# speechcatcher-asr/statecatcher

Hardware: AMD Instinct MI355X
Metric: audio-frames/sec (LucyRNN+CTC, 80-d fbank, T=1500), whole job (higher is better)
Workload: dtype bf16

## Files before the change

### statecatcher_amd/csrc/lucy_scan.hip

```cpp

#include <atomic>
#include <initializer_list>
#include <type_traits>

#include "sc_common.h"

namespace sc {


constexpr int kChunk = 64;
typedef uint32_t v4u __attribute__((ext_vector_type(4)));
constexpr float kEps = 1e-6f;

struct ScanFwdArgs {
  const void* gates;
  const float* bias;
  const float* h0;
  const float* s0;
  void* out;
  float* s_out;
  float* h_out;
  float* ckpt;
  int B, T, D, nsc;
  int64_t g_bt, g_td, g_cd, g_cb, o_bt, o_bd;
  void* out_dup;
  void* out_lo;
  const float* ln_r;
  const float2* rec_in;
  float2* ln_stat;
  float2* rec_out;
  float ln_eps;
};

struct ScanBwdArgs {
  const void* gates;
  const float* bias;
  const float* ckpt;
  const void* dout;
  const float* ds_last;
  void* dgates;
  float* dh0;
  float* ds0;
  float* dbias;
  int B, T, D, nsc;
  int64_t g_bt, g_td, g_cd, g_cb, d_bt, d_bd, dg_bt, dg_td, dg_cd, dg_cb;
  const float* ln_r;
  const float2* ln_stat;
};

template <typename T, int PW> struct Pieces {
  static constexpr int EPP = PW / (int)sizeof(T);
  static constexpr int PPR = 64 / EPP;
  static_assert(EPP >= 1 && 64 % EPP == 0, "piece width");
};
template <typename T, int PW> struct LdsElem {
  static constexpr int BYTES = PW == 2 ? 4 : (int)sizeof(T);
  static __device__ __forceinline__ T get(const unsigned char* slot, int idx) {
    return *(const T*)(slot + idx * BYTES);
  }
};

__device__ __forceinline__ void step_terms(float r, float z, float k, float v, float hp, float dc,
                                           float al, float& zg, float& dec, float& u, float& hn) {
  const float rc2 = (r * r + z * z) * 0.5f + kEps;
  const float q = (k * k + v * v) * 0.5f + kEps;
  zg = sigm(z * rsq(rc2));
  dec = sigm(dc * rsq(dc * dc + kEps));
  const float alp = sigm(al * rsq(al * al + kEps));
  hn = hp * rsq(hp * hp + kEps);
  const float iq = rsq(q);
  const float kv = (k * iq) * (v * iq) * rcp(q + kEps);
  u = alp * kv;
}

typedef float f2 __attribute__((ext_vector_type(2)));
__device__ __forceinline__ f2 rsq2(f2 x) { return f2{rsq(x.x), rsq(x.y)}; }
__device__ __forceinline__ f2 rcp2(f2 x) { return f2{rcp(x.x), rcp(x.y)}; }
__device__ __forceinline__ f2 sigm2(f2 x) {
  const f2 t = x * f2{-kLog2e, -kLog2e};
  return rcp2(f2{1.0f, 1.0f} + f2{exp2_(t.x), exp2_(t.y)});
}
__device__ __forceinline__ f2 tanh2(f2 x) {
  const f2 t = x * f2{-2.0f * kLog2e, -2.0f * kLog2e};
  const f2 r = rcp2(f2{1.0f, 1.0f} + f2{exp2_(t.x), exp2_(t.y)});
  return r + r - f2{1.0f, 1.0f};
}
template <int DT> struct Pair {
  using T = typename Elem<DT>::T;
  typedef T t2 __attribute__((ext_vector_type(2)));
  static __device__ __forceinline__ t2 st(f2 v) { return __builtin_convertvector(v, t2); }
};

__device__ __forceinline__ void step_terms2(f2 r, f2 z, f2 k, f2 v, f2 hp, f2 dc, f2 al, f2& zg,
                                            f2& dec, f2& u, f2& hn) {
  const f2 eps = {kEps, kEps}, half = {0.5f, 0.5f};
  const f2 rc2 = (r * r + z * z) * half + eps;
  const f2 q = (k * k + v * v) * half + eps;
  zg = sigm2(z * rsq2(rc2));
  dec = sigm2(dc * rsq2(dc * dc + eps));
  const f2 alp = sigm2(al * rsq2(al * al + eps));
  hn = hp * rsq2(hp * hp + eps);
  const f2 iq = rsq2(q);
  u = alp * ((k * iq) * (v * iq) * rcp2(q + eps));
}

__device__ __forceinline__ float tanh_sig(float x) { return sigm(2.0f * x) * 2.0f - 1.0f; }

__device__ __forceinline__ void gate_grads(float r, float z, float k, float v, float hp, float dc,
                                           float al, float zg, float dec, float gh, float dpre,
                                           float gs, float hprev, float sprev, float c,
                                           float (&o)[7]) {
  const float rc2 = (r * r + z * z) * 0.5f + kEps;
  const float irc = rsq(rc2);
  const float ird = rsq(dc * dc + kEps);
  const float ira = rsq(al * al + kEps);
  const float alp = sigm(al * ira);
  const float irh = rsq(hp * hp + kEps);
  const float q = (k * k + v * v) * 0.5f + kEps;
  const float iq = rsq(q);
  const float iqe = rcp(q + kEps);
  const float d_zn = gh * (hprev - c) * zg * (1.0f - zg) * (irc * irc * irc);
  o[0] = -d_zn * z * r * 0.5f;
  o[1] = d_zn * (r * r * 0.5f + kEps);
  const float d_kv = gs * alp;
  const float f = iq * iq * iqe;
  const float fp = -(2.0f * q + kEps) * f * f;
  o[2] = d_kv * v * (f + k * k * fp);
  o[3] = d_kv * k * (f + v * v * fp);
  o[4] = dpre * kEps * (irh * irh * irh);
  o[5] = gs * sprev * dec * (1.0f - dec) * kEps * (ird * ird * ird);
  o[6] = gs * (k * v * f) * alp * (1.0f - alp) * kEps * (ira * ira * ira);
}


__device__ __forceinline__ void gate_grads2(f2 r, f2 z, f2 k, f2 v, f2 hp, f2 dc, f2 al, f2 zg,
                                            f2 dec, f2 gh, f2 dpre, f2 gs, f2 hprev, f2 sprev,
                                            f2 c, f2 (&o)[7]) {
  const f2 one = {1.0f, 1.0f}, eps = {kEps, kEps}, half = {0.5f, 0.5f};
  const f2 rc2 = (r * r + z * z) * half + eps;
  const f2 irc = rsq2(rc2);
  const f2 ird = rsq2(dc * dc + eps);
  const f2 ira = rsq2(al * al + eps);
  const f2 alp = sigm2(al * ira);
  const f2 irh = rsq2(hp * hp + eps);
  const f2 q = (k * k + v * v) * half + eps;
  const f2 iq = rsq2(q);
  const f2 iqe = rcp2(q + eps);
  const f2 d_zn = gh * (hprev - c) * zg * (one - zg) * (irc * irc * irc);
  o[0] = -d_zn * z * r * half;
  o[1] = d_zn * (r * r * half + eps);
  const f2 d_kv = gs * alp;
  const f2 f = iq * iq * iqe;
  const f2 fp = -(q + q + eps) * f * f;
  o[2] = d_kv * v * (f + k * k * fp);
  o[3] = d_kv * k * (f + v * v * fp);
  o[4] = dpre * eps * (irh * irh * irh);
  o[5] = gs * sprev * dec * (one - dec) * eps * (ird * ird * ird);
  o[6] = gs * (k * v * f) * alp * (one - alp) * eps * (ira * ira * ira);
}

__device__ __forceinline__ void step_terms_bwd2(f2 r, f2 z, f2 k, f2 v, f2 hp, f2 dc, f2 al,
                                                f2& zg, f2& dec, f2& u, f2& hn, f2 (&cf)[7]) {
  const f2 one = {1.0f, 1.0f}, eps = {kEps, kEps}, half = {0.5f, 0.5f};
  const f2 rc2 = (r * r + z * z) * half + eps;
  const f2 q = (k * k + v * v) * half + eps;
  const f2 irc = rsq2(rc2);
  zg = sigm2(z * irc);
  const f2 ird = rsq2(dc * dc + eps);
  dec = sigm2(dc * ird);
  const f2 ira = rsq2(al * al + eps);
  const f2 alp = sigm2(al * ira);
  const f2 irh = rsq2(hp * hp + eps);
  hn = hp * irh;
  const f2 iq = rsq2(q);
  const f2 f = iq * iq * rcp2(q + eps);
  const f2 kv = k * v * f;
  u = alp * kv;
  const f2 kz = zg * (one - zg) * (irc * irc * irc);
  cf[0] = -kz * z * r * half;
  cf[1] = kz * (r * r * half + eps);
  const f2 fp = -(q + q + eps) * f * f;
  cf[2] = alp * v * (f + k * k * fp);
  cf[3] = alp * k * (f + v * v * fp);
  cf[4] = eps * (irh * irh * irh);
  cf[5] = dec * (one - dec) * eps * (ird * ird * ird);
  cf[6] = kv * alp * (one - alp) * eps * (ira * ira * ira);
}

template <int NW>
__device__ __forceinline__ float compose_prefix(const float2 (*agg)[64], int lane, int w, float x) {
  int q = 0;
  for (; q + 4 <= w; q += 4) {
    const float2 m0 = agg[q][lane], m1 = agg[q + 1][lane], m2 = agg[q + 2][lane],
                 m3 = agg[q + 3][lane];
    x = fmaf(m0.x, x, m0.y);
    x = fmaf(m1.x, x, m1.y);
    x = fmaf(m2.x, x, m2.y);
    x = fmaf(m3.x, x, m3.y);
  }
  for (; q < w; ++q) {
    const float2 m = agg[q][lane];
    x = fmaf(m.x, x, m.y);
  }
  return x;
}
template <int NW>
__device__ __forceinline__ float compose_suffix(const float2 (*agg)[64], int lane, int w, float x) {
  int q = NW - 1;
  for (; q - 4 >= w; q -= 4) {
    const float2 m0 = agg[q][lane], m1 = agg[q - 1][lane], m2 = agg[q - 2][lane],
                 m3 = agg[q - 3][lane];
    x = fmaf(m0.x, x, m0.y);
    x = fmaf(m1.x, x, m1.y);
    x = fmaf(m2.x, x, m2.y);
    x = fmaf(m3.x, x, m3.y);
  }
  for (; q > w; --q) {
    const float2 m = agg[q][lane];
    x = fmaf(m.x, x, m.y);
  }
  return x;
}

template <int N>
__device__ __forceinline__ float group_sum_dpp(float x) {
  static_assert(N == 2 || N == 4 || N == 8 || N == 16, "group of 2..16 lanes");
  x = dpp_step<0xB1, 0xf, false>(x);
  if constexpr (N >= 4) x = dpp_step<0x4E, 0xf, false>(x);
  if constexpr (N >= 8) x = dpp_step<0x141, 0xf, false>(x);
  if constexpr (N >= 16) x = dpp_step<0x140, 0xf, false>(x);
  return x;
}

template <int DT, int NW, int LC, int PW, int FD, bool SPLIT = false, int LN = 0, int NB = 8>
__global__ void __launch_bounds__(NW * 64)
lucy_scan_fwd_kernel(ScanFwdArgs a) {
  static_assert(NW * LC == kChunk, "super-chunk must be 64 steps");
  using E = Elem<DT>;
  using T = typename E::T;
  using P = Pieces<T, PW>;
  constexpr int ROWS = LC * 7;
  constexpr int PIECES = ROWS * P::PPR;
  constexpr int NI = (PIECES + 63) / 64;
  const int lane = threadIdx.x & 63;
  const int w = uniform(threadIdx.x >> 6);
  const int b = blockIdx.y;
  const int blk = blockIdx.x;
  const int d = blk * 64 + lane;
  const bool dok = d < a.D;
  const int dc = dok ? d : a.D - 1;
  const int pcmax = (min(64, a.D - blk * 64) - 1) / P::EPP;

  extern __shared__ __attribute__((aligned(16))) unsigned char dyn_lds[];
  __shared__ float2 aggS[NW][64];
  __shared__ float2 aggH[NW][64];
  __shared__ float carS[2][64];
  __shared__ float carH[2][64];
  constexpr int RECN = (LN & 1) ? LC * NB : 2;
  static_assert(!(LN & 1) || (RECN <= 64 && NB % 2 == 0), "LN fold: LC * NB <= 64, NB even");
  __shared__ __attribute__((aligned(16))) float2 recS[(LN & 1) ? FD : 1][(LN & 1) ? NW : 1][RECN];
  using L = LdsElem<T, PW>;
  constexpr int SLOTB = ROWS * 64 * L::BYTES;
  const unsigned char* slots = dyn_lds + w * FD * SLOTB;
  const uint32_t slots_lds = lds_addr(slots);

  const T* gsrc = (const T*)a.gates + (int64_t)b * a.g_bt + (int64_t)blk * a.g_cb;
  const Buf<T> obuf((T*)a.out + (int64_t)b * a.o_bt);
  const Buf<T> dbuf(SPLIT ? (T*)a.out_dup + (int64_t)b * a.o_bt : (T*)a.out);
  const Buf<T> lbuf(SPLIT ? (T*)a.out_lo + (int64_t)b * a.o_bt : (T*)a.out);
  const uint32_t vo = (uint32_t)d * sizeof(T);
  const uint32_t otd = (uint32_t)(a.o_bd * sizeof(T));
  if (w == 0) {
    carS[0][lane] = dok ? a.s0[(int64_t)b * a.D + d] : 0.0f;
    carH[0][lane] = dok ? a.h0[(int64_t)b * a.D + d] : 0.0f;
  }
  float gb[7], fr[7];
#pragma unroll
  for (int g = 0; g < 7; ++g) {
    gb[g] = a.bias ? a.bias[g * a.D + dc] : 0.0f;
    fr[g] = (LN & 1) ? a.ln_r[g * a.D + dc] : 0.0f;
  }
  settle(gb);
  settle(fr);
  const int Tm1 = a.T - 1;
  auto issue_rec = [&](int k) __attribute__((always_inline)) {
    if constexpr ((LN & 1) != 0) {
      constexpr int NP = LC * NB / 2;
      if (lane < NP) {
        const int j = lane / (NB / 2), q2 = lane % (NB / 2);
        const int t = min(k * kChunk + w * LC + j, Tm1);
        dma_to_lds<16>(a.rec_in + ((int64_t)b * a.T + t) * NB + 2 * q2,
                       lds_addr(&recS[(LN & 1) ? k % FD : 0][(LN & 1) ? w : 0][0]));
      }
    }
  };
  auto issue = [&](int k) __attribute__((always_inline)) {
    issue_rec(k);
#pragma unroll
    for (int i = 0; i < NI; ++i) {
      const int p = i * 64 + lane;
      if (PIECES % 64 == 0 || p < PIECES) {
        const int row = p / P::PPR, pc = p % P::PPR;
        const int j = row / 7, g = row - 7 * (row / 7);
        const int t = min(k * kChunk + w * LC + j, Tm1);
        dma_to_lds<PW>(gsrc + (int64_t)t * a.g_td + (int64_t)g * a.g_cd + min(pc, pcmax) * P::EPP,
                       slots_lds + (uint32_t)((k % FD) * SLOTB) + i * 64 * (PW == 2 ? 4 : PW));
      }
    }
  };
  constexpr bool kFast = NI <= 16;
  uint32_t voff[kFast ? NI : 1];
#pragma unroll
  for (int i = 0; i < (kFast ? NI : 0); ++i) {
    const int p = min(i * 64 + lane, PIECES - 1);
    const int row = p / P::PPR, pc = p % P::PPR;
    voff[i] = (uint32_t)((row / 7) * a.g_td + (row % 7) * a.g_cd + min(pc, pcmax) * P::EPP) *
              (uint32_t)sizeof(T);
  }
  auto issue_next = [&](int k) __attribute__((always_inline)) {
    if (kFast && (k + 1) * kChunk <= a.T) {
      issue_rec(k);
      const T* gt = gsrc + ((int64_t)k * kChunk + w * LC) * a.g_td;
#pragma unroll
      for (int i = 0; i < (kFast ? NI : 0); ++i)
        if (PIECES % 64 == 0 || i * 64 + lane < PIECES)
          dma_to_lds_s<PW>(gt, voff[i], slots_lds + (uint32_t)((k % FD) * SLOTB) + i * 64 * (PW == 2 ? 4 : PW));
    } else {
      issue(k);
    }
  };
  constexpr int NIR = NI + ((LN & 1) ? 1 : 0);
  auto wait_next = [&](int k) __attribute__((always_inline)) {
    if (FD == 2 && k + 2 < a.nsc) dma_wait_younger<NIR>();
    else dma_wait();
  };
  if (a.nsc > 0) issue(0);
  if (FD == 2 && a.nsc > 1) issue(1);
  wait_next(-1);
  lds_barrier();
  auto chunk = [&](int k, auto fullc) __attribute__((always_inline)) {
    constexpr bool FULL = decltype(fullc)::value;
    constexpr int LP = LC / 2;
    const int t0 = k * kChunk + w * LC;
    f2 zg[LP], dec[LP], u[LP], x[LP], wz[LP];
    float gv[LC][7];
    const unsigned char* slot = slots + (k % FD) * SLOTB;
    if constexpr ((LN & 1) != 0) {
      const float2 rq = recS[(LN & 1) ? k % FD : 0][(LN & 1) ? w : 0][lane % RECN];
      const float mean = group_sum_dpp<NB>(rq.x) * (1.0f / NB);
      const float dm = rq.x - mean;
      const float m2 = group_sum_dpp<NB>(fmaf(64.0f * dm, dm, rq.y));
      const float rstd = rsq(m2 * (1.0f / (64 * NB)) + a.ln_eps);
      if (a.ln_stat && blk == 0 && lane % NB == 0 && lane < RECN && k * kChunk + w * LC + lane / NB < a.T)
        a.ln_stat[(int64_t)b * a.T + k * kChunk + w * LC + lane / NB] = make_float2(rstd, mean);
#pragma unroll
      for (int j = 0; j < LC; ++j) {
        const float rs = __int_as_float(__builtin_amdgcn_readlane(__float_as_int(rstd), j * NB));
        const float mu = __int_as_float(__builtin_amdgcn_readlane(__float_as_int(mean), j * NB));
        const float rm = -rs * mu;
#pragma unroll
        for (int g = 0; g < 7; ++g)
          gv[j][g] = fmaf(E::ld(L::get(slot, (j * 7 + g) * 64 + lane)), rs, fmaf(rm, fr[g], gb[g]));
      }
    } else {
#pragma unroll
      for (int j = 0; j < LC; ++j)
#pragma unroll
        for (int g = 0; g < 7; ++g) gv[j][g] = E::ld(L::get(slot, (j * 7 + g) * 64 + lane)) + gb[g];
    }
    lds_read_wait();
    if (k + FD < a.nsc) issue_next(k + FD);
#pragma unroll
    for (int p = 0; p < LP; ++p) {
      const int j = 2 * p;
      step_terms2(f2{gv[j][0], gv[j + 1][0]}, f2{gv[j][1], gv[j + 1][1]},
                  f2{gv[j][2], gv[j + 1][2]}, f2{gv[j][3], gv[j + 1][3]},
                  f2{gv[j][4], gv[j + 1][4]}, f2{gv[j][5], gv[j + 1][5]},
                  f2{gv[j][6], gv[j + 1][6]}, zg[p], dec[p], u[p], x[p]);
      if constexpr (!FULL) {
#pragma unroll
        for (int h2 = 0; h2 < 2; ++h2) {
          if (t0 + j + h2 >= a.T) {
            zg[p][h2] = 1.0f; dec[p][h2] = 1.0f; u[p][h2] = 0.0f; x[p][h2] = 0.0f;
          }
        }
      }
    }
    float As = 1.0f, Bs = 0.0f;
#pragma unroll
    for (int j = 0; j < LC; ++j) {
      As *= dec[j >> 1][j & 1];
      Bs = fmaf(dec[j >> 1][j & 1], Bs, u[j >> 1][j & 1]);
    }
    aggS[w][lane] = make_float2(As, Bs);
    lds_barrier();
    float s = carS[k & 1][lane];
    const float s_in = s;
    s = compose_prefix<NW>(aggS, lane, w, s);
#pragma unroll
    for (int j = 0; j < LC; ++j) {
      s = fmaf(dec[j >> 1][j & 1], s, u[j >> 1][j & 1]);
      x[j >> 1][j & 1] += s;
    }
#pragma unroll
    for (int p = 0; p < LP; ++p) {
      x[p] = tanh2(x[p]);
      wz[p] = x[p] - zg[p] * x[p];
    }
    float Ah = 1.0f, Bh = 0.0f;
#pragma unroll
    for (int j = 0; j < LC; ++j) {
      Ah *= zg[j >> 1][j & 1];
      Bh = fmaf(zg[j >> 1][j & 1], Bh, wz[j >> 1][j & 1]);
    }
    if (w == NW - 1) carS[(k + 1) & 1][lane] = s;
    aggH[w][lane] = make_float2(Ah, Bh);
    lds_barrier();
    float h = carH[k & 1][lane];
    const float h_in = h;
    h = compose_prefix<NW>(aggH, lane, w, h);
    float hs[LC];
#pragma unroll
    for (int j = 0; j < LC; ++j) {
      h = fmaf(zg[j >> 1][j & 1], h, wz[j >> 1][j & 1]);
      hs[j] = h;
    }
    if (w == NW - 1) carH[(k + 1) & 1][lane] = h;
    wait_next(k);
    if (w == 0 && a.ckpt && dok) {
      a.ckpt[((int64_t)(b * a.nsc + k) * 2) * a.D + d] = s_in;
      a.ckpt[((int64_t)(b * a.nsc + k) * 2 + 1) * a.D + d] = h_in;
    }
#pragma unroll
    for (int j = 0; j < LC; ++j)
      if (FULL || (dok && t0 + j < a.T)) {
        const T hi = E::st(hs[j]);
        obuf.st(hi, vo, (uint32_t)(t0 + j) * otd);
        if constexpr (SPLIT) {
          dbuf.st(hi, vo, (uint32_t)(t0 + j) * otd);
          lbuf.st(E::st(hs[j] - E::ld(hi)), vo, (uint32_t)(t0 + j) * otd);
        }
      }
    if constexpr ((LN & 2) != 0) {
      static_assert(LC == 4, "record butterfly written for 4 steps per wave");
      float v[8], ref[LC];
#pragma unroll
      for (int j = 0; j < LC; ++j) {
        const float hb = E::ld(E::st(hs[j]));
        ref[j] = __int_as_float(__builtin_amdgcn_readfirstlane(__float_as_int(hb)));
        const float dl = hb - ref[j];
        v[2 * j] = dl;
        v[2 * j + 1] = dl * dl;
      }
      const bool b5 = lane & 32, b4 = lane & 16, b3 = lane & 8;
      float u4[4], u2[2];
#pragma unroll
      for (int i = 0; i < 4; ++i)
        u4[i] = (b5 ? v[i + 4] : v[i]) + __shfl_xor(b5 ? v[i] : v[i + 4], 32);
#pragma unroll
      for (int i = 0; i < 2; ++i)
        u2[i] = (b4 ? u4[i + 2] : u4[i]) + __shfl_xor(b4 ? u4[i] : u4[i + 2], 16);
      float y = (b3 ? u2[1] : u2[0]) + __shfl_xor(b3 ? u2[0] : u2[1], 8);
      y = group_sum_dpp<8>(y);
      const float ysq = __shfl_xor(y, 8);
      const int j = lane >> 4;
      const float r = j == 0 ? ref[0] : j == 1 ? ref[1] : j == 2 ? ref[2] : ref[3];
      if ((lane & 15) == 0 && t0 + j < a.T)
        a.rec_out[((int64_t)b * a.T + t0 + j) * NB + blk] =
            make_float2(fmaf(y, 1.0f / 64, r), fmaxf(ysq - y * y * (1.0f / 64), 0.0f));
    }
  };
  const bool blk_full = (blk + 1) * 64 <= a.D;
  for (int k = 0; k < a.nsc; ++k) {
    if (blk_full && (k + 1) * kChunk <= a.T)
      chunk(k, std::true_type{});
    else
      chunk(k, std::false_type{});
  }
  lds_barrier();
  if (w == 0 && dok) {
    a.s_out[(int64_t)b * a.D + d] = carS[a.nsc & 1][lane];
    if (a.h_out) a.h_out[(int64_t)b * a.D + d] = carH[a.nsc & 1][lane];
  }
}

template <int DT, int NW, int LC, int PW, int NBUF, bool WST, int LN = 0>
__global__ void __launch_bounds__(NW * 64)
lucy_scan_bwd_kernel(ScanBwdArgs a) {
  static_assert(NW * LC == kChunk, "super-chunk must be 64 steps");
  using E = Elem<DT>;
  using T = typename E::T;
  using P = Pieces<T, PW>;
  constexpr int GROWS = LC * 7;
  constexpr int ROWS = LC * 8;
  constexpr int PIECES = ROWS * P::PPR;
  constexpr int NI = (PIECES + 63) / 64;
  static_assert(!WST || (NBUF == 2 && PW == 16), "staged stores need two 16-bit slots");
  const int lane = threadIdx.x & 63;
  const int w = uniform(threadIdx.x >> 6);
  const int b = blockIdx.y;
  const int blk = blockIdx.x;
  const int d = blk * 64 + lane;
  const bool dok = d < a.D;
  const int dc = dok ? d : a.D - 1;
  const int pcmax = (min(64, a.D - blk * 64) - 1) / P::EPP;

  extern __shared__ __attribute__((aligned(16))) unsigned char dyn_lds[];
  __shared__ float2 aggA[NW][64];
  __shared__ float2 aggB[NW][64];
  __shared__ float2 aggC[NW][64];
  __shared__ float2 aggD[NW][64];
  __shared__ float carGh[2][64];
  __shared__ float carGs[2][64];
  __shared__ float ckS[2][2][64];
  static_assert(!LN || (NBUF == 2 && WST), "LN fold: 16-bit gates with staged stores");
  __shared__ __attribute__((aligned(16))) float2 stS[LN ? NBUF : 1][LN ? NW : 1][LN ? LC : 1];
  using L = LdsElem<T, PW>;
  unsigned char* slots = dyn_lds + w * NBUF * ROWS * 64 * L::BYTES;
  const uint32_t slots_lds = lds_addr(slots);

  const T* gsrc = (const T*)a.gates + (int64_t)b * a.g_bt + (int64_t)blk * a.g_cb;
  const T* dsrc = (const T*)a.dout + (int64_t)b * a.d_bt + (int64_t)blk * 64;
  const float* cksrc = a.ckpt + (int64_t)b * a.nsc * 2 * a.D + dc;
  const Buf<T> dgbuf((T*)a.dgates + (int64_t)b * a.dg_bt + (int64_t)blk * a.dg_cb);
  const uint32_t vo = (uint32_t)lane * sizeof(T);
  if (w == 0) {
    carGh[0][lane] = 0.0f;
    carGs[0][lane] = (a.ds_last && dok) ? a.ds_last[(int64_t)b * a.D + d] : 0.0f;
  }
  float gb[LN ? 1 : 7];
  __shared__ float2 fbS[LN ? 7 : 1][64];
  if constexpr (LN) {
    if (w < 7)
      fbS[LN ? w : 0][lane] = make_float2(a.bias[w * a.D + dc], LN == 1 ? a.ln_r[w * a.D + dc] : 0.0f);
  } else {
#pragma unroll
    for (int g = 0; g < 7; ++g) gb[g] = a.bias ? a.bias[g * a.D + dc] : 0.0f;
    settle(gb);
  }
  const int Tm1 = a.T - 1;
  auto issue_stat = [&](int it) __attribute__((always_inline)) {
    if constexpr (LN) {
      if (lane < 2 * LC) {
        const int k = a.nsc - 1 - it;
        const int t = min(k * kChunk + w * LC + (lane >> 1), Tm1);
        dma_to_lds<4>((const float*)(a.ln_stat + (int64_t)b * a.T + t) + (lane & 1),
                      lds_addr(&stS[LN ? it % NBUF : 0][LN ? w : 0][0]));
      }
    }
  };
  auto issue = [&](int it) __attribute__((always_inline)) {
    const int k = a.nsc - 1 - it;
    issue_stat(it);
    const uint32_t base = slots_lds + (uint32_t)((it % NBUF) * ROWS * 64 * L::BYTES);
#pragma unroll
    for (int i = 0; i < NI; ++i) {
      const int p = i * 64 + lane;
      if (PIECES % 64 == 0 || p < PIECES) {
        const int row = p / P::PPR, pc = p % P::PPR;
        const int col = min(pc, pcmax) * P::EPP;
        const T* src;
        if (row < GROWS) {
          const int j = row / 7, g = row - 7 * (row / 7);
          const int t = min(k * kChunk + w * LC + j, Tm1);
          src = gsrc + (int64_t)t * a.g_td + (int64_t)g * a.g_cd + col;
        } else {
          const int t = min(k * kChunk + w * LC + (row - GROWS), Tm1);
          src = dsrc + (int64_t)t * a.d_bd + col;
        }
        dma_to_lds<PW>(src, base + i * 64 * (PW == 2 ? 4 : PW));
      }
    }
    if (w == 0) {
      dma_to_lds<4>(cksrc + (int64_t)(k * 2) * a.D, lds_addr(&ckS[it & 1][0][0]));
      dma_to_lds<4>(cksrc + (int64_t)(k * 2 + 1) * a.D, lds_addr(&ckS[it & 1][1][0]));
    }
  };
  static_assert((GROWS * P::PPR) % 64 == 0 && PIECES % 64 == 0, "uniform row kind per DMA");
  constexpr int NIF = NI <= 16 ? NI : 1;
  const bool same_layout = NI <= 16 && a.dg_td == a.g_td && a.dg_cd == a.g_cd;
  __shared__ uint32_t voffT[NIF][64];
  if constexpr (NI <= 16) {
#pragma unroll
    for (int i = 0; i < NI; ++i) {
      if (i % NW != w) continue;
      const int p = i * 64 + lane;
      const int row = p / P::PPR, pc = p % P::PPR;
      const int col = min(pc, pcmax) * P::EPP;
      voffT[i][lane] = (uint32_t)(row < GROWS ? (row / 7) * a.g_td + (row % 7) * a.g_cd + col
                                              : (row - GROWS) * a.d_bd + col) *
                       (uint32_t)sizeof(T);
    }
  }
  auto issue_full = [&](int it) __attribute__((always_inline)) {
    const int k = a.nsc - 1 - it;
    issue_stat(it);
    const uint32_t base = slots_lds + (uint32_t)((it % NBUF) * ROWS * 64 * L::BYTES);
    const int64_t t = (int64_t)k * kChunk + w * LC;
    const T* gt = gsrc + t * a.g_td;
    const T* dt = dsrc + t * a.d_bd;
#pragma unroll
    for (int i = 0; i < NI; ++i)
      dma_to_lds_s<PW>((i * 64) / P::PPR < GROWS ? (const void*)gt : (const void*)dt, voffT[i][lane],
                       base + i * 64 * (PW == 2 ? 4 : PW));
    if (w == 0) {
      const float* ck = a.ckpt + ((int64_t)b * a.nsc + k) * 2 * a.D;
      dma_to_lds_s<4>(ck, (uint32_t)dc * 4u, lds_addr(&ckS[it & 1][0][0]));
      dma_to_lds_s<4>(ck + a.D, (uint32_t)dc * 4u, lds_addr(&ckS[it & 1][1][0]));
    }
  };
  auto issue_next = [&](int it) __attribute__((always_inline)) {
    if constexpr (NI <= 16) issue_full(it); else issue(it);
  };
  f2 bacc[7];
  float bacc1[7];
#pragma unroll
  for (int g = 0; g < 7; ++g) {
    bacc[g] = f2{0.0f, 0.0f};
    bacc1[g] = 0.0f;
  }
  if (a.nsc > 0) issue(0);
  dma_wait();
  lds_barrier();
  auto chunk = [&](int it, auto fullc) __attribute__((always_inline)) {
    constexpr bool FULL = decltype(fullc)::value;
    constexpr int LP = LC / 2;
    const int k = a.nsc - 1 - it;
    const int t0 = k * kChunk + w * LC;
    unsigned char* slot = slots + (it % NBUF) * ROWS * 64 * L::BYTES;
    if (NBUF == 2 && it + 1 < a.nsc) issue_next(it + 1);
    const float s_ck = ckS[it & 1][0][lane];
    const float h_ck = ckS[it & 1][1][lane];
    f2 zg[LP], dec[LP], u[LP], x[LP], dj[LP], sv[LP], hv[LP], wz[LP];
    f2 cf[LP][7];
    float rg[NBUF == 1 ? LC : 1][7];
#pragma unroll
    for (int p = 0; p < LP; ++p) {
      const int j = 2 * p;
      f2 g7[7];
      f2 lrs = {1.0f, 1.0f}, lrm = {0.0f, 0.0f};
      if constexpr (LN) {
        const float2 s0 = stS[LN ? it % NBUF : 0][LN ? w : 0][j];
        const float2 s1 = stS[LN ? it % NBUF : 0][LN ? w : 0][j + 1];
        lrs = f2{s0.x, s1.x};
        lrm = -lrs * f2{s0.y, s1.y};
      }
#pragma unroll
      for (int g = 0; g < 7; ++g) {
        const f2 raw = f2{E::ld(L::get(slot, (j * 7 + g) * 64 + lane)),
                          E::ld(L::get(slot, ((j + 1) * 7 + g) * 64 + lane))};
        if constexpr (LN == 1) {
          const float2 fb = fbS[LN ? g : 0][lane];
          g7[g] = raw * lrs + (lrm * f2{fb.y, fb.y} + f2{fb.x, fb.x});
        } else if constexpr (LN == 2) {
          const float fbx = fbS[LN ? g : 0][lane].x;
          g7[g] = raw + f2{fbx, fbx};
        } else {
          g7[g] = raw + gb[LN ? 0 : g];
        }
        if constexpr (NBUF == 1) {
          rg[j][g] = g7[g].x;
          rg[j + 1][g] = g7[g].y;
        }
      }
      if constexpr (NBUF == 2)
        step_terms_bwd2(g7[0], g7[1], g7[2], g7[3], g7[4], g7[5], g7[6], zg[p], dec[p], u[p],
                        x[p], cf[p]);
      else
        step_terms2(g7[0], g7[1], g7[2], g7[3], g7[4], g7[5], g7[6], zg[p], dec[p], u[p], x[p]);
      dj[p] = f2{E::ld(L::get(slot, (GROWS + j) * 64 + lane)),
                 E::ld(L::get(slot, (GROWS + j + 1) * 64 + lane))};
      if constexpr (!FULL) {
#pragma unroll
        for (int h2 = 0; h2 < 2; ++h2) {
          if (t0 + j + h2 >= a.T) {
            zg[p][h2] = 1.0f; dec[p][h2] = 1.0f; u[p][h2] = 0.0f; x[p][h2] = 0.0f;
            dj[p][h2] = 0.0f;
          }
        }
      }
    }
    f2* stash = (f2*)slot;
    if constexpr (NBUF == 2) {
#pragma unroll
      for (int p = 0; p < LP; ++p)
#pragma unroll
        for (int c = 0; c < 4; ++c) stash[(p * 4 + c) * 64 + lane] = cf[p][c];
    }
    float As = 1.0f, Bs = 0.0f;
#pragma unroll
    for (int j = 0; j < LC; ++j) {
      As *= dec[j >> 1][j & 1];
      Bs = fmaf(dec[j >> 1][j & 1], Bs, u[j >> 1][j & 1]);
    }
    if constexpr (NBUF == 1) {
      lds_read_wait();
      if (it + 1 < a.nsc) issue_next(it + 1);
    }
    float Ph = 1.0f, Qh = 0.0f;
#pragma unroll
    for (int j = LC - 1; j >= 0; --j) {
      Qh = zg[j >> 1][j & 1] * (dj[j >> 1][j & 1] + Qh);
      Ph *= zg[j >> 1][j & 1];
    }
    aggA[w][lane] = make_float2(As, Bs);
    aggC[w][lane] = make_float2(Ph, Qh);
    lds_barrier();
    float s = compose_prefix<NW>(aggA, lane, w, s_ck);
#pragma unroll
    for (int j = 0; j < LC; ++j) {
      sv[j >> 1][j & 1] = s;
      s = fmaf(dec[j >> 1][j & 1], s, u[j >> 1][j & 1]);
      x[j >> 1][j & 1] += s;
    }
#pragma unroll
    for (int p = 0; p < LP; ++p) {
      x[p] = tanh2(x[p]);
      wz[p] = x[p] - zg[p] * x[p];
      if constexpr (NBUF == 2) cf[p][5] *= sv[p];
    }
    float Ah = 1.0f, Bh = 0.0f;
#pragma unroll
    for (int j = 0; j < LC; ++j) {
      Ah *= zg[j >> 1][j & 1];
      Bh = fmaf(zg[j >> 1][j & 1], Bh, wz[j >> 1][j & 1]);
    }
    float C = compose_suffix<NW>(aggC, lane, w, carGh[it & 1][lane]);
#pragma unroll
    for (int j = LC - 1; j >= 0; --j) {
      u[j >> 1][j & 1] = dj[j >> 1][j & 1] + C;
      C = zg[j >> 1][j & 1] * u[j >> 1][j & 1];
    }
    if (w == 0) carGh[(it + 1) & 1][lane] = C;
    f2 dp[LP];
#pragma unroll
    for (int p = 0; p < LP; ++p) dp[p] = (u[p] - u[p] * zg[p]) * (f2{1.0f, 1.0f} - x[p] * x[p]);
    float Ps = 1.0f, Qs = 0.0f;
#pragma unroll
    for (int j = LC - 1; j >= 0; --j) {
      Qs = dec[j >> 1][j & 1] * (dp[j >> 1][j & 1] + Qs);
      Ps *= dec[j >> 1][j & 1];
    }
    aggB[w][lane] = make_float2(Ah, Bh);
    aggD[w][lane] = make_float2(Ps, Qs);
    dma_wait();
    lds_barrier();
    float h = compose_prefix<NW>(aggB, lane, w, h_ck);
#pragma unroll
    for (int j = 0; j < LC; ++j) {
      if constexpr (NBUF == 2)
        hv[j >> 1][j & 1] = u[j >> 1][j & 1] * (h - x[j >> 1][j & 1]);
      else
        hv[j >> 1][j & 1] = h;
      h = fmaf(zg[j >> 1][j & 1], h, wz[j >> 1][j & 1]);
    }
    float Cs = compose_suffix<NW>(aggD, lane, w, carGs[it & 1][lane]);
    f2 gsj[LP];
#pragma unroll
    for (int j = LC - 1; j >= 0; --j) {
      gsj[j >> 1][j & 1] = dp[j >> 1][j & 1] + Cs;
      Cs = dec[j >> 1][j & 1] * gsj[j >> 1][j & 1];
    }
#pragma unroll
    for (int p = 0; p < LP; ++p) {
      const int jp = 2 * p;
      f2 o[7];
      if constexpr (NBUF == 2) {
        const f2 gz = hv[p];
        o[0] = gz * stash[(p * 4 + 0) * 64 + lane];
        o[1] = gz * stash[(p * 4 + 1) * 64 + lane];
        o[2] = gsj[p] * stash[(p * 4 + 2) * 64 + lane];
        o[3] = gsj[p] * stash[(p * 4 + 3) * 64 + lane];
        o[4] = dp[p] * cf[p][4];
        o[5] = gsj[p] * cf[p][5];
        o[6] = gsj[p] * cf[p][6];
      } else {
        f2 g7[7];
#pragma unroll
        for (int g = 0; g < 7; ++g) g7[g] = f2{rg[jp][g], rg[jp + 1][g]};
        gate_grads2(g7[0], g7[1], g7[2], g7[3], g7[4], g7[5], g7[6], zg[p], dec[p], u[p], dp[p],
                    gsj[p], hv[p], sv[p], x[p], o);
      }
      if constexpr (FULL && NBUF == 2) {
#pragma unroll
        for (int g = 0; g < 7; ++g) bacc[g] += o[g];
      }
      f2 lrs = {1.0f, 1.0f};
      if constexpr (LN) {
        lrs = f2{stS[LN ? it % NBUF : 0][LN ? w : 0][jp].x, stS[LN ? it % NBUF : 0][LN ? w : 0][jp + 1].x};
        if constexpr (FULL) {
#pragma unroll
          for (int g = 0; g < 7; ++g) o[g] *= lrs;
        }
      }
      if constexpr (FULL && WST) {
#pragma unroll
        for (int g = 0; g < 7; ++g) {
          const auto pr = Pair<DT>::st(o[g]);
          ((T*)slot)[(jp * 7 + g) * 64 + lane] = pr.x;
          ((T*)slot)[((jp + 1) * 7 + g) * 64 + lane] = pr.y;
        }
      } else {
#pragma unroll
        for (int h2 = 0; h2 < 2; ++h2) {
          const int j = jp + h2;
          if (FULL || (dok && t0 + j < a.T)) {
            const uint32_t so = (uint32_t)((t0 + j) * a.dg_td * sizeof(T));
#pragma unroll
            for (int g = 0; g < 7; ++g) {
              const float og = o[g][h2];
              const T ogt = E::st(LN ? og * lrs[h2] : og);
              if constexpr (WST) ((T*)slot)[(j * 7 + g) * 64 + lane] = ogt;
              else dgbuf.st(ogt, vo, so + (uint32_t)(g * a.dg_cd * sizeof(T)));
              if constexpr (NBUF == 1) bacc1[g] += E::ld(ogt);
              else if constexpr (!FULL) bacc[g][h2] += og;
            }
          }
        }
      }
    }
    if constexpr (WST) {
      constexpr int SP = LC * 7 * 8;
#pragma unroll
      for (int i = 0; i < (SP + 63) / 64; ++i) {
        const int p = i * 64 + lane;
        if (SP % 64 == 0 || p < SP) {
          const int row = p >> 3, pc = p & 7;
          const int j = row / 7, g = row - 7 * (row / 7);
          if (FULL || (t0 + j < a.T && pc <= pcmax)) {
            const v4u v = *(const v4u*)(slot + p * 16);
            if constexpr (FULL)
              __builtin_amdgcn_raw_buffer_store_b128(v, dgbuf.r, voffT[i][lane],
                                                     (uint32_t)(t0 * a.dg_td * sizeof(T)), 0);
            else
              __builtin_amdgcn_raw_buffer_store_b128(
                  v, dgbuf.r,
                  ((uint32_t)(t0 + j) * (uint32_t)a.dg_td + (uint32_t)g * (uint32_t)a.dg_cd +
                   (uint32_t)pc * 8u) * (uint32_t)sizeof(T),
                  0, 0);
          }
        }
      }
    }
    if (w == 0) carGs[(it + 1) & 1][lane] = Cs;
  };
  const bool blk_full = (blk + 1) * 64 <= a.D && (!WST || same_layout);
  for (int it = 0; it < a.nsc; ++it) {
    if constexpr (NBUF == 2) {
      if (blk_full && (a.nsc - it) * kChunk <= a.T) {
        chunk(it, std::true_type{});
        continue;
      }
    }
    chunk(it, std::false_type{});
  }
  lds_barrier();
  if (w == 0 && dok) {
    a.dh0[(int64_t)b * a.D + d] = carGh[a.nsc & 1][lane];
    a.ds0[(int64_t)b * a.D + d] = carGs[a.nsc & 1][lane];
  }
  if (a.dbias) {
#pragma unroll
    for (int g = 0; g < 7; ++g) {
      aggA[w][lane].x = NBUF == 1 ? bacc1[g] : bacc[g].x + bacc[g].y;
      lds_barrier();
      if (w == 0) {
        float acc = 0.0f;
        for (int q = 0; q < NW; ++q) acc += aggA[q][lane].x;
        if (dok) a.dbias[((int64_t)b * 7 + g) * a.D + d] = acc;
      }
      lds_barrier();
    }
  }
}

constexpr int kNW = 16, kLC = kChunk / kNW;
constexpr int kBNW = 8, kBLC = kChunk / kBNW;

template <typename K>
static bool set_lds_limit(K kernel, size_t bytes) {
  return hipFuncSetAttribute((const void*)kernel, hipFuncAttributeMaxDynamicSharedMemorySize,
                             (int)bytes) == hipSuccess;
}

template <int DT, int PW, bool SPLIT = false, int LN = 0, int NB = 8>
static void launch_fwd(const ScanFwdArgs& a, hipStream_t st) {
  using T = typename Elem<DT>::T;
  constexpr int FD = 1;
  auto kern = lucy_scan_fwd_kernel<DT, kNW, kLC, PW, FD, SPLIT, LN, NB>;
  const size_t lds = (size_t)FD * kNW * kLC * 7 * 64 * LdsElem<T, PW>::BYTES;
  static const bool lds_ok = set_lds_limit(kern, lds);
  (void)lds_ok;
  dim3 grid((a.D + 63) / 64, a.B);
  hipLaunchKernelGGL(kern, grid, dim3(kNW * 64), lds, st, a);
}

template <int DT, int PW, bool WST, int LN = 0>
static void launch_bwd(const ScanBwdArgs& a, hipStream_t st) {
  using T = typename Elem<DT>::T;
  constexpr int NBUF = LdsElem<T, PW>::BYTES == 2 ? 2 : 1;
  auto kern = lucy_scan_bwd_kernel<DT, kBNW, kBLC, PW, NBUF, WST, LN>;
  const size_t lds = (size_t)NBUF * kBNW * kBLC * 8 * 64 * LdsElem<T, PW>::BYTES;
  static const bool lds_ok = set_lds_limit(kern, lds);
  (void)lds_ok;
  dim3 grid((a.D + 63) / 64, a.B);
  hipLaunchKernelGGL(kern, grid, dim3(kBNW * 64), lds, st, a);
}

static bool wide_pieces(const void* p, int esize, int D, std::initializer_list<int64_t> strides) {
  const int epp = 16 / esize;
  if ((uintptr_t)p % 16 || D % epp) return false;
  for (int64_t s : strides)
    if (s % epp) return false;
  return true;
}

template <int DT, bool SPLIT, int NB>
static void dispatch_fwd_ln(const ScanFwdArgs& a, int mode, hipStream_t st) {
  switch (mode) {
    case 1: launch_fwd<DT, 16, SPLIT, 1, NB>(a, st); break;
    case 2: launch_fwd<DT, 16, SPLIT, 2, NB>(a, st); break;
    default: launch_fwd<DT, 16, SPLIT, 3, NB>(a, st); break;
  }
}
template <int DT, bool SPLIT>
static void dispatch_fwd_ln_nb(const ScanFwdArgs& a, int mode, hipStream_t st) {
  if (a.D == 512) dispatch_fwd_ln<DT, SPLIT, 8>(a, mode, st);
  else dispatch_fwd_ln<DT, SPLIT, 16>(a, mode, st);
}

template <int DT>
static void dispatch_fwd(const ScanFwdArgs& a, hipStream_t st) {
  constexpr int es = (int)sizeof(typename Elem<DT>::T);
  const bool wide = wide_pieces(a.gates, es, a.D, {a.g_bt, a.g_td, a.g_cd, a.g_cb});
  if constexpr (es == 2) {
    const int mode = (a.ln_r ? 1 : 0) | (a.rec_out ? 2 : 0);
    if (mode) {
      if (a.out_lo) dispatch_fwd_ln_nb<DT, true>(a, mode, st);
      else dispatch_fwd_ln_nb<DT, false>(a, mode, st);
      return;
    }
    if (a.out_lo) {
      if (wide) launch_fwd<DT, 16, true>(a, st);
      else launch_fwd<DT, es, true>(a, st);
      return;
    }
  }
  if (wide) launch_fwd<DT, 16>(a, st);
  else launch_fwd<DT, es>(a, st);
}

template <int DT>
static void dispatch_bwd(const ScanBwdArgs& a, hipStream_t st) {
  constexpr int es = sizeof(typename Elem<DT>::T);
  if constexpr (es == 2) {
    if (a.ln_stat) {
      if (a.ln_r) launch_bwd<DT, 16, true, 1>(a, st);
      else launch_bwd<DT, 16, true, 2>(a, st);
      return;
    }
  }
  if (wide_pieces(a.gates, es, a.D, {a.g_bt, a.g_td, a.g_cd, a.g_cb}) &&
      wide_pieces(a.dout, es, a.D, {a.d_bt, a.d_bd})) {
    if (es == 2 && wide_pieces(a.dgates, es, a.D, {a.dg_bt, a.dg_td, a.dg_cd, a.dg_cb}))
      launch_bwd<DT, 16, es == 2>(a, st);
    else
      launch_bwd<DT, 16, false>(a, st);
  } else {
    launch_bwd<DT, es, false>(a, st);
  }
}

}

using namespace sc;

extern "C" int sc_lucy_scan_chunk(void) { return kChunk; }

extern "C" int64_t sc_lucy_scan_ckpt_numel(int B, int T, int D) {
  if (B < 0 || T < 0 || D < 0) return 0;
  return (int64_t)B * ((T + kChunk - 1) / kChunk) * 2 * D;
}

static int check_dtype(int dt) { return dt == SC_F32 || dt == SC_BF16 || dt == SC_F16; }

struct LnFold {
  const float* r = nullptr;
  const float* rec_in = nullptr;
  float* stat = nullptr;
  float* rec_out = nullptr;
  float eps = 1e-5f;
};

static int scan_fwd(const void* gates, int gates_dtype, const float* gate_bias, const float* h0,
                    const float* s0, void* out, float* s_out, float* h_out, int B, int T, int D,
                    int64_t stride_g_bt, int64_t stride_g_td, int64_t stride_g_cd,
                    int64_t stride_g_cb, int64_t stride_o_bt, int64_t stride_o_bd, float* ckpt,
// ... 164 lines not shown
```

Baseline: 9.231 million.

## Split per-wave chunk into two half-sequences scanned in packed f2 lanes

Time steps within a wave are re-paired so each f2 holds step p and step p+LP. This lets the intra-chunk linear recurrences (decay/state, gate/hidden, and the backward suffix scans) run as two independent half-length chains in packed float2 math, with the halves joined by one fma. The kv normalisation is simplified from rsq*rsq*rcp to a single rcp of q*(q+eps), and the backward stash is given a custom row layout checked at compile time. The change shortens the serial dependency chain and cuts transcendental work, but it reorders floating-point rounding and hard-codes an 8-step-per-wave stash assumption.

```diff
diff --git a/statecatcher_amd/csrc/lucy_scan.hip b/statecatcher_amd/csrc/lucy_scan.hip
--- a/statecatcher_amd/csrc/lucy_scan.hip
+++ b/statecatcher_amd/csrc/lucy_scan.hip
@@ -68,8 +68,7 @@
   dec = sigm(dc * rsq(dc * dc + kEps));
   const float alp = sigm(al * rsq(al * al + kEps));
   hn = hp * rsq(hp * hp + kEps);
-  const float iq = rsq(q);
-  const float kv = (k * iq) * (v * iq) * rcp(q + kEps);
+  const float kv = k * v * rcp(q * (q + kEps));
   u = alp * kv;
 }
 
@@ -100,8 +99,7 @@
   dec = sigm2(dc * rsq2(dc * dc + eps));
   const f2 alp = sigm2(al * rsq2(al * al + eps));
   hn = hp * rsq2(hp * hp + eps);
-  const f2 iq = rsq2(q);
-  u = alp * ((k * iq) * (v * iq) * rcp2(q + eps));
+  u = alp * (k * v * rcp2(q * (q + eps)));
 }
 
 __device__ __forceinline__ float tanh_sig(float x) { return sigm(2.0f * x) * 2.0f - 1.0f; }
@@ -117,13 +115,11 @@
   const float alp = sigm(al * ira);
   const float irh = rsq(hp * hp + kEps);
   const float q = (k * k + v * v) * 0.5f + kEps;
-  const float iq = rsq(q);
-  const float iqe = rcp(q + kEps);
   const float d_zn = gh * (hprev - c) * zg * (1.0f - zg) * (irc * irc * irc);
   o[0] = -d_zn * z * r * 0.5f;
   o[1] = d_zn * (r * r * 0.5f + kEps);
   const float d_kv = gs * alp;
-  const float f = iq * iq * iqe;
+  const float f = rcp(q * (q + kEps));
   const float fp = -(2.0f * q + kEps) * f * f;
   o[2] = d_kv * v * (f + k * k * fp);
   o[3] = d_kv * k * (f + v * v * fp);
@@ -144,13 +140,11 @@
   const f2 alp = sigm2(al * ira);
   const f2 irh = rsq2(hp * hp + eps);
   const f2 q = (k * k + v * v) * half + eps;
-  const f2 iq = rsq2(q);
-  const f2 iqe = rcp2(q + eps);
   const f2 d_zn = gh * (hprev - c) * zg * (one - zg) * (irc * irc * irc);
   o[0] = -d_zn * z * r * half;
   o[1] = d_zn * (r * r * half + eps);
   const f2 d_kv = gs * alp;
-  const f2 f = iq * iq * iqe;
+  const f2 f = rcp2(q * (q + eps));
   const f2 fp = -(q + q + eps) * f * f;
   o[2] = d_kv * v * (f + k * k * fp);
   o[3] = d_kv * k * (f + v * v * fp);
@@ -172,8 +166,7 @@
   const f2 alp = sigm2(al * ira);
   const f2 irh = rsq2(hp * hp + eps);
   hn = hp * irh;
-  const f2 iq = rsq2(q);
-  const f2 f = iq * iq * rcp2(q + eps);
+  const f2 f = rcp2(q * (q + eps));
   const f2 kv = k * v * f;
   u = alp * kv;
   const f2 kz = zg * (one - zg) * (irc * irc * irc);
@@ -372,59 +365,64 @@
     if (k + FD < a.nsc) issue_next(k + FD);
 #pragma unroll
     for (int p = 0; p < LP; ++p) {
-      const int j = 2 * p;
-      step_terms2(f2{gv[j][0], gv[j + 1][0]}, f2{gv[j][1], gv[j + 1][1]},
-                  f2{gv[j][2], gv[j + 1][2]}, f2{gv[j][3], gv[j + 1][3]},
-                  f2{gv[j][4], gv[j + 1][4]}, f2{gv[j][5], gv[j + 1][5]},
-                  f2{gv[j][6], gv[j + 1][6]}, zg[p], dec[p], u[p], x[p]);
+      const int j = p, jh = p + LP;
+      step_terms2(f2{gv[j][0], gv[jh][0]}, f2{gv[j][1], gv[jh][1]},
+                  f2{gv[j][2], gv[jh][2]}, f2{gv[j][3], gv[jh][3]},
+                  f2{gv[j][4], gv[jh][4]}, f2{gv[j][5], gv[jh][5]},
+                  f2{gv[j][6], gv[jh][6]}, zg[p], dec[p], u[p], x[p]);
       if constexpr (!FULL) {
 #pragma unroll
         for (int h2 = 0; h2 < 2; ++h2) {
-          if (t0 + j + h2 >= a.T) {
+          if (t0 + p + h2 * LP >= a.T) {
             zg[p][h2] = 1.0f; dec[p][h2] = 1.0f; u[p][h2] = 0.0f; x[p][h2] = 0.0f;
           }
         }
       }
     }
-    float As = 1.0f, Bs = 0.0f;
-#pragma unroll
-    for (int j = 0; j < LC; ++j) {
-      As *= dec[j >> 1][j & 1];
-      Bs = fmaf(dec[j >> 1][j & 1], Bs, u[j >> 1][j & 1]);
-    }
-    aggS[w][lane] = make_float2(As, Bs);
+    f2 Pd = dec[0], Bs2 = u[0];
+#pragma unroll
+    for (int p = 1; p < LP; ++p) {
+      Pd *= dec[p];
+      Bs2 = dec[p] * Bs2 + u[p];
+    }
+    aggS[w][lane] = make_float2(Pd.y * Pd.x, fmaf(Pd.y, Bs2.x, Bs2.y));
     lds_barrier();
     float s = carS[k & 1][lane];
     const float s_in = s;
     s = compose_prefix<NW>(aggS, lane, w, s);
-#pragma unroll
-    for (int j = 0; j < LC; ++j) {
-      s = fmaf(dec[j >> 1][j & 1], s, u[j >> 1][j & 1]);
-      x[j >> 1][j & 1] += s;
-    }
+    f2 s2 = {s, fmaf(Pd.x, s, Bs2.x)};
+#pragma unroll
+    for (int p = 0; p < LP; ++p) {
+      s2 = dec[p] * s2 + u[p];
+      x[p] += s2;
+    }
+    s = s2.y;
 #pragma unroll
     for (int p = 0; p < LP; ++p) {
       x[p] = tanh2(x[p]);
       wz[p] = x[p] - zg[p] * x[p];
     }
-    float Ah = 1.0f, Bh = 0.0f;
-#pragma unroll
-    for (int j = 0; j < LC; ++j) {
-      Ah *= zg[j >> 1][j & 1];
-      Bh = fmaf(zg[j >> 1][j & 1], Bh, wz[j >> 1][j & 1]);
+    f2 Pz = zg[0], Bh2 = wz[0];
+#pragma unroll
+    for (int p = 1; p < LP; ++p) {
+      Pz *= zg[p];
+      Bh2 = zg[p] * Bh2 + wz[p];
     }
     if (w == NW - 1) carS[(k + 1) & 1][lane] = s;
-    aggH[w][lane] = make_float2(Ah, Bh);
+    aggH[w][lane] = make_float2(Pz.y * Pz.x, fmaf(Pz.y, Bh2.x, Bh2.y));
     lds_barrier();
     float h = carH[k & 1][lane];
     const float h_in = h;
     h = compose_prefix<NW>(aggH, lane, w, h);
+    f2 h2 = {h, fmaf(Pz.x, h, Bh2.x)};
     float hs[LC];
 #pragma unroll
-    for (int j = 0; j < LC; ++j) {
-      h = fmaf(zg[j >> 1][j & 1], h, wz[j >> 1][j & 1]);
-      hs[j] = h;
-    }
+    for (int p = 0; p < LP; ++p) {
+      h2 = zg[p] * h2 + wz[p];
+      hs[p] = h2.x;
+      hs[p + LP] = h2.y;
+    }
+    h = h2.y;
     if (w == NW - 1) carH[(k + 1) & 1][lane] = h;
     wait_next(k);
     if (w == 0 && a.ckpt && dok) {
@@ -482,6 +480,27 @@
     a.s_out[(int64_t)b * a.D + d] = carS[a.nsc & 1][lane];
     if (a.h_out) a.h_out[(int64_t)b * a.D + d] = carH[a.nsc & 1][lane];
   }
+}
+
+constexpr int stash_row(int p, int c) {
+  const int nlow = p < 3 ? 2 : 1;
+  return c < nlow ? 4 * (2 * p + c) : 28 + 4 * (2 * p + c - nlow);
+}
+constexpr bool stash_layout_ok() {
+  for (int q = 0; q < 16; ++q) {
+    const int r = stash_row(q / 4, q % 4);
+    if (r < 0 || r + 4 > 64) return false;
+    for (int q2 = 0; q2 < q; ++q2) {
+      const int r2 = stash_row(q2 / 4, q2 % 4);
+      if (r < r2 + 4 && r2 < r + 4) return false;
+    }
+    for (int p = 0; p < q / 4; ++p)
+      for (int half = 0; half < 2; ++half) {
+        const int g0 = 7 * (p + 4 * half);
+        if (r < g0 + 7 && g0 < r + 4) return false;
+      }
+  }
+  return true;
 }
 
 template <int DT, int NW, int LC, int PW, int NBUF, bool WST, int LN = 0>
@@ -629,26 +648,24 @@
     const int t0 = k * kChunk + w * LC;
     unsigned char* slot = slots + (it % NBUF) * ROWS * 64 * L::BYTES;
     if (NBUF == 2 && it + 1 < a.nsc) issue_next(it + 1);
-    const float s_ck = ckS[it & 1][0][lane];
-    const float h_ck = ckS[it & 1][1][lane];
     f2 zg[LP], dec[LP], u[LP], x[LP], dj[LP], sv[LP], hv[LP], wz[LP];
     f2 cf[LP][7];
     float rg[NBUF == 1 ? LC : 1][7];
 #pragma unroll
     for (int p = 0; p < LP; ++p) {
-      const int j = 2 * p;
+      const int j = p, jh = p + LP;
       f2 g7[7];
       f2 lrs = {1.0f, 1.0f}, lrm = {0.0f, 0.0f};
       if constexpr (LN) {
         const float2 s0 = stS[LN ? it % NBUF : 0][LN ? w : 0][j];
-        const float2 s1 = stS[LN ? it % NBUF : 0][LN ? w : 0][j + 1];
+        const float2 s1 = stS[LN ? it % NBUF : 0][LN ? w : 0][jh];
         lrs = f2{s0.x, s1.x};
         lrm = -lrs * f2{s0.y, s1.y};
       }
 #pragma unroll
       for (int g = 0; g < 7; ++g) {
         const f2 raw = f2{E::ld(L::get(slot, (j * 7 + g) * 64 + lane)),
-                          E::ld(L::get(slot, ((j + 1) * 7 + g) * 64 + lane))};
+                          E::ld(L::get(slot, (jh * 7 + g) * 64 + lane))};
         if constexpr (LN == 1) {
           const float2 fb = fbS[LN ? g : 0][lane];
           g7[g] = raw * lrs + (lrm * f2{fb.y, fb.y} + f2{fb.x, fb.x});
@@ -660,7 +677,7 @@
         }
         if constexpr (NBUF == 1) {
           rg[j][g] = g7[g].x;
-          rg[j + 1][g] = g7[g].y;
+          rg[jh][g] = g7[g].y;
         }
       }
       if constexpr (NBUF == 2)
@@ -669,11 +686,11 @@
       else
         step_terms2(g7[0], g7[1], g7[2], g7[3], g7[4], g7[5], g7[6], zg[p], dec[p], u[p], x[p]);
       dj[p] = f2{E::ld(L::get(slot, (GROWS + j) * 64 + lane)),
-                 E::ld(L::get(slot, (GROWS + j + 1) * 64 + lane))};
+                 E::ld(L::get(slot, (GROWS + jh) * 64 + lane))};
       if constexpr (!FULL) {
 #pragma unroll
         for (int h2 = 0; h2 < 2; ++h2) {
-          if (t0 + j + h2 >= a.T) {
+          if (t0 + p + h2 * LP >= a.T) {
             zg[p][h2] = 1.0f; dec[p][h2] = 1.0f; u[p][h2] = 0.0f; x[p][h2] = 0.0f;
             dj[p][h2] = 0.0f;
           }
@@ -682,36 +699,40 @@
     }
     f2* stash = (f2*)slot;
     if constexpr (NBUF == 2) {
+      static_assert(LC == 8 && stash_layout_ok(), "cf0-3 stash laid out for 8 steps per wave");
 #pragma unroll
       for (int p = 0; p < LP; ++p)
 #pragma unroll
-        for (int c = 0; c < 4; ++c) stash[(p * 4 + c) * 64 + lane] = cf[p][c];
-    }
-    float As = 1.0f, Bs = 0.0f;
-#pragma unroll
-    for (int j = 0; j < LC; ++j) {
-      As *= dec[j >> 1][j & 1];
-      Bs = fmaf(dec[j >> 1][j & 1], Bs, u[j >> 1][j & 1]);
+        for (int c = 0; c < 4; ++c) stash[stash_row(p, c) * 16 + lane] = cf[p][c];
+    }
+    f2 Pd = dec[0], Bs2 = u[0];
+#pragma unroll
+    for (int p = 1; p < LP; ++p) {
+      Pd *= dec[p];
+      Bs2 = dec[p] * Bs2 + u[p];
     }
     if constexpr (NBUF == 1) {
       lds_read_wait();
       if (it + 1 < a.nsc) issue_next(it + 1);
     }
-    float Ph = 1.0f, Qh = 0.0f;
-#pragma unroll
-    for (int j = LC - 1; j >= 0; --j) {
-      Qh = zg[j >> 1][j & 1] * (dj[j >> 1][j & 1] + Qh);
-      Ph *= zg[j >> 1][j & 1];
-    }
-    aggA[w][lane] = make_float2(As, Bs);
-    aggC[w][lane] = make_float2(Ph, Qh);
+    f2 Pz = zg[LP - 1], Qh2 = zg[LP - 1] * dj[LP - 1];
+#pragma unroll
+    for (int p = LP - 2; p >= 0; --p) {
+      Qh2 = zg[p] * (dj[p] + Qh2);
+      Pz *= zg[p];
+    }
+    aggA[w][lane] = make_float2(Pd.y * Pd.x, fmaf(Pd.y, Bs2.x, Bs2.y));
+    aggC[w][lane] = make_float2(Pz.y * Pz.x, fmaf(Pz.x, Qh2.y, Qh2.x));
     lds_barrier();
-    float s = compose_prefix<NW>(aggA, lane, w, s_ck);
-#pragma unroll
-    for (int j = 0; j < LC; ++j) {
-      sv[j >> 1][j & 1] = s;
-      s = fmaf(dec[j >> 1][j & 1], s, u[j >> 1][j & 1]);
-      x[j >> 1][j & 1] += s;
+    const float s_ck = ckS[it & 1][0][lane];
+    const float h_ck = ckS[it & 1][1][lane];
+    const float s = compose_prefix<NW>(aggA, lane, w, s_ck);
+    f2 s2 = {s, fmaf(Pd.x, s, Bs2.x)};
+#pragma unroll
+    for (int p = 0; p < LP; ++p) {
+      sv[p] = s2;
+      s2 = dec[p] * s2 + u[p];
+      x[p] += s2;
     }
 #pragma unroll
     for (int p = 0; p < LP; ++p) {
@@ -719,65 +740,62 @@
       wz[p] = x[p] - zg[p] * x[p];
       if constexpr (NBUF == 2) cf[p][5] *= sv[p];
     }
-    float Ah = 1.0f, Bh = 0.0f;
-#pragma unroll
-    for (int j = 0; j < LC; ++j) {
-      Ah *= zg[j >> 1][j & 1];
-      Bh = fmaf(zg[j >> 1][j & 1], Bh, wz[j >> 1][j & 1]);
-    }
-    float C = compose_suffix<NW>(aggC, lane, w, carGh[it & 1][lane]);
-#pragma unroll
-    for (int j = LC - 1; j >= 0; --j) {
-      u[j >> 1][j & 1] = dj[j >> 1][j & 1] + C;
-      C = zg[j >> 1][j & 1] * u[j >> 1][j & 1];
-    }
-    if (w == 0) carGh[(it + 1) & 1][lane] = C;
+    f2 Bh2 = wz[0];
+#pragma unroll
+    for (int p = 1; p < LP; ++p) Bh2 = zg[p] * Bh2 + wz[p];
+    const float C = compose_suffix<NW>(aggC, lane, w, carGh[it & 1][lane]);
+    f2 C2 = {fmaf(Pz.y, C, Qh2.y), C};
+#pragma unroll
+    for (int p = LP - 1; p >= 0; --p) {
+      u[p] = dj[p] + C2;
+      C2 = zg[p] * u[p];
+    }
+    if (w == 0) carGh[(it + 1) & 1][lane] = C2.x;
     f2 dp[LP];
 #pragma unroll
     for (int p = 0; p < LP; ++p) dp[p] = (u[p] - u[p] * zg[p]) * (f2{1.0f, 1.0f} - x[p] * x[p]);
-    float Ps = 1.0f, Qs = 0.0f;
-#pragma unroll
-    for (int j = LC - 1; j >= 0; --j) {
-      Qs = dec[j >> 1][j & 1] * (dp[j >> 1][j & 1] + Qs);
-      Ps *= dec[j >> 1][j & 1];
-    }
-    aggB[w][lane] = make_float2(Ah, Bh);
-    aggD[w][lane] = make_float2(Ps, Qs);
+    f2 Qs2 = dec[LP - 1] * dp[LP - 1];
+#pragma unroll
+    for (int p = LP - 2; p >= 0; --p) Qs2 = dec[p] * (dp[p] + Qs2);
+    aggB[w][lane] = make_float2(Pz.y * Pz.x, fmaf(Pz.y, Bh2.x, Bh2.y));
+    aggD[w][lane] = make_float2(Pd.y * Pd.x, fmaf(Pd.x, Qs2.y, Qs2.x));
     dma_wait();
     lds_barrier();
-    float h = compose_prefix<NW>(aggB, lane, w, h_ck);
-#pragma unroll
-    for (int j = 0; j < LC; ++j) {
+    const float h = compose_prefix<NW>(aggB, lane, w, h_ck);
+    f2 hh = {h, fmaf(Pz.x, h, Bh2.x)};
+#pragma unroll
+    for (int p = 0; p < LP; ++p) {
       if constexpr (NBUF == 2)
-        hv[j >> 1][j & 1] = u[j >> 1][j & 1] * (h - x[j >> 1][j & 1]);
+        hv[p] = u[p] * (hh - x[p]);
       else
-        hv[j >> 1][j & 1] = h;
-      h = fmaf(zg[j >> 1][j & 1], h, wz[j >> 1][j & 1]);
-    }
-    float Cs = compose_suffix<NW>(aggD, lane, w, carGs[it & 1][lane]);
+        hv[p] = hh;
+      hh = zg[p] * hh + wz[p];
+    }
+    const float Cs = compose_suffix<NW>(aggD, lane, w, carGs[it & 1][lane]);
+    f2 Cs2 = {fmaf(Pd.y, Cs, Qs2.y), Cs};
     f2 gsj[LP];
 #pragma unroll
-    for (int j = LC - 1; j >= 0; --j) {
-      gsj[j >> 1][j & 1] = dp[j >> 1][j & 1] + Cs;
-      Cs = dec[j >> 1][j & 1] * gsj[j >> 1][j & 1];
+    for (int p = LP - 1; p >= 0; --p) {
+      gsj[p] = dp[p] + Cs2;
+      Cs2 = dec[p] * gsj[p];
     }
 #pragma unroll
     for (int p = 0; p < LP; ++p) {
-      const int jp = 2 * p;
+      const int jl = p, jh = p + LP;
       f2 o[7];
       if constexpr (NBUF == 2) {
         const f2 gz = hv[p];
-        o[0] = gz * stash[(p * 4 + 0) * 64 + lane];
-        o[1] = gz * stash[(p * 4 + 1) * 64 + lane];
-        o[2] = gsj[p] * stash[(p * 4 + 2) * 64 + lane];
-        o[3] = gsj[p] * stash[(p * 4 + 3) * 64 + lane];
+        o[0] = gz * stash[stash_row(p, 0) * 16 + lane];
+        o[1] = gz * stash[stash_row(p, 1) * 16 + lane];
+        o[2] = gsj[p] * stash[stash_row(p, 2) * 16 + lane];
+        o[3] = gsj[p] * stash[stash_row(p, 3) * 16 + lane];
         o[4] = dp[p] * cf[p][4];
         o[5] = gsj[p] * cf[p][5];
         o[6] = gsj[p] * cf[p][6];
       } else {
         f2 g7[7];
 #pragma unroll
-        for (int g = 0; g < 7; ++g) g7[g] = f2{rg[jp][g], rg[jp + 1][g]};
+        for (int g = 0; g < 7; ++g) g7[g] = f2{rg[jl][g], rg[jh][g]};
         gate_grads2(g7[0], g7[1], g7[2], g7[3], g7[4], g7[5], g7[6], zg[p], dec[p], u[p], dp[p],
                     gsj[p], hv[p], sv[p], x[p], o);
       }
@@ -787,7 +805,7 @@
       }
       f2 lrs = {1.0f, 1.0f};
       if constexpr (LN) {
-        lrs = f2{stS[LN ? it % NBUF : 0][LN ? w : 0][jp].x, stS[LN ? it % NBUF : 0][LN ? w : 0][jp + 1].x};
+        lrs = f2{stS[LN ? it % NBUF : 0][LN ? w : 0][jl].x, stS[LN ? it % NBUF : 0][LN ? w : 0][jh].x};
         if constexpr (FULL) {
 #pragma unroll
           for (int g = 0; g < 7; ++g) o[g] *= lrs;
@@ -797,13 +815,13 @@
 #pragma unroll
         for (int g = 0; g < 7; ++g) {
           const auto pr = Pair<DT>::st(o[g]);
-          ((T*)slot)[(jp * 7 + g) * 64 + lane] = pr.x;
-          ((T*)slot)[((jp + 1) * 7 + g) * 64 + lane] = pr.y;
+          ((T*)slot)[(jl * 7 + g) * 64 + lane] = pr.x;
+          ((T*)slot)[(jh * 7 + g) * 64 + lane] = pr.y;
         }
       } else {
 #pragma unroll
         for (int h2 = 0; h2 < 2; ++h2) {
-          const int j = jp + h2;
+          const int j = h2 ? jh : jl;
           if (FULL || (dok && t0 + j < a.T)) {
             const uint32_t so = (uint32_t)((t0 + j) * a.dg_td * sizeof(T));
 #pragma unroll
@@ -842,7 +860,7 @@
         }
       }
     }
-    if (w == 0) carGs[(it + 1) & 1][lane] = Cs;
+    if (w == 0) carGs[(it + 1) & 1][lane] = Cs2.x;
   };
   const bool blk_full = (blk + 1) * 64 <= a.D && (!WST || same_layout);
   for (int it = 0; it < a.nsc; ++it) {
```

Result: no change. 9.317 million (median of 6 runs) (+0.9%).
